# xiyichen/smplify-x-partial

Hardware: AMD Instinct MI355X
Metric: fitted frames/sec (higher is better)
Workload: dtype f32; 1 GPU; configs[1]: 256 synthetic frames/GPU, body-only K=25, camera + 5-stage L-BFGS (fit_smplx_smplifyx.yaml, use_vposer=False); frames_per_gpu=256, lbs_mode=dense, gemm_columns_per_gpu=256, parallelism=frames sharded, dp1, closure_evals_per_frame_max=4429, non_finite=0

## Files before the change

### smplify-x-partial_amd/csrc/closure_body.h

```cpp
#pragma once
#include "closure_math.h"
#include "closure_lds.h"
#pragma clang fp contract(on)

#define MARK(i) do { if (D.dbg && blockIdx.x == 0 && threadIdx.x == 0 && D.dbg[62] <= D.dbg[61]) { D.dbg[i] = clock64(); \
        if ((i) == 0) D.dbg[17] = wall_clock64(); if ((i) == 16) D.dbg[18] = wall_clock64(); } } while (0)

#define FOR_CT(w, N) _Pragma("unroll") for (int w##_i = 0; w##_i < ((N) + CT - 1) / CT; ++w##_i)             \
                         if (const int w = t + w##_i * CT; w < (N))

struct NoUpstream {};
struct ExtUpstream {
    const float* djoints;
    int has_dverts;
    float* gc;
};

struct OwnOperands {
    __device__ __forceinline__ int tid() const { return threadIdx.x; }
    __device__ __forceinline__ const float* featR(const BatchDev& D) const { return D.featR; }
    __device__ __forceinline__ float* featR_w(const BatchDev& D) const { return D.featR_w; }
    __device__ __forceinline__ float* AT_w(const BatchDev& D) const { return D.AT_w; }
};
struct OperandSets {
    const float* r; float* fw; float* aw; int t;
    __device__ __forceinline__ int tid() const { return t; }
    __device__ __forceinline__ const float* featR(const BatchDev&) const { return r; }
    __device__ __forceinline__ float* featR_w(const BatchDev&) const { return fw; }
    __device__ __forceinline__ float* AT_w(const BatchDev&) const { return aw; }
};

template <class LDS, class SW, class EXT = NoUpstream, class OPS = OwnOperands>
__device__ __forceinline__ void closure_body(LDS& S, const DevModel& M, const BatchDev& D,
                                             const VarList* __restrict__ vls, const SW* __restrict__ sws,
                                             const ClosureArgs& args, const int b, typename LDS::real_t* gflat,
                                             typename LDS::real_t* fout, const EXT& ext = EXT{}, const OPS ops = OPS{}) {
    using Real = typename LDS::real_t;
    constexpr bool F64 = std::is_same<Real, double>::value;
    constexpr bool kExt = !std::is_same<EXT, NoUpstream>::value;
    static_assert(!kExt || !F64, "the external-upstream sweep is fp32");
    constexpr int CT = LDS::kThreads;
    const int t = ops.tid();
    const int lane = t & 63, wv = t >> 6;
    const ParLayout& L = D.L;
    const BatchCfgDev& C = D.cfg;

    const bool self_uvp = !F64 && args.use_dense_verts == 2 && M.n_uniq > 0 && M.n_uniq <= LDS::kMaxItems;
    const int stage = __builtin_amdgcn_readfirstlane((args.stage_override != -2) ? args.stage_override : D.stage[b]);
    if constexpr (!kExt) { if (stage >= C.n_stages && !args.forward_only) return; }
    const bool cam_stage = (stage < 0);
    const SW sw = (kExt || cam_stage || args.forward_only) ? SW{} : sws[stage];

    const int cls = (kExt || cam_stage || args.forward_only) ? 2 : ((sw.face_jw != 0.f) ? 2 : ((sw.hand_jw != 0.f) ? 1 : 0));
    const int KL = __builtin_amdgcn_readfirstlane(cls == 2 ? M.K : C.kl[cls]);
    const int NIL = __builtin_amdgcn_readfirstlane(cls == 2 ? M.n_items : C.nil[cls]);

    MARK(0);
    constexpr bool HAS_VP = !std::is_same<decltype(S.V), EmptyLDS>::value;
    constexpr int RIF = (LDS::kMaxItems <= SFX_SMALL_ITEMS) ? SFX_RIF_SMALL : SFX_RIF_BIG;
    constexpr int FWD_PREFIX = (int)(offsetof(LDS, vp) / sizeof(float));
    static_assert(F64 || (FWD_PREFIX % 4 == 0 && FWD_PREFIX + 96 + 2 * VP_H + 128 + 64 <= SFX_FWD_N), "forward-state blob layout");
    static_assert(offsetof(LDS, Ad) % sizeof(fwd_t) == 0 && offsetof(LDS, cd) % sizeof(fwd_t) == 0, "forward-precision members");
    const bool reuse = !F64 && args.reuse_fwd != 0;
    float* fwd = D.fwd ? D.fwd + (size_t)b * SFX_FWD_N : nullptr;
    const Real* xsrc;
    if constexpr (F64) xsrc = (args.from_X ? D.X64 : D.Xt64) + (size_t)b * SFX_NPAR_MAX;
    else xsrc = (args.from_X ? D.X : D.Xt) + (size_t)b * SFX_NPAR_MAX;
    if (!reuse) {
        if (args.x_lds) { for (int i = t; i < L.npar; i += CT) S.x[i] = args.x_lds[i]; }
        else lds_fill_async<CT>(S.x, xsrc, L.npar * (int)(sizeof(Real) / 4));
    }
    if (!args.keep_tables) {
    static_assert(SFX_META_N % 4 == 0 && FD_N % 4 == 0 && offsetof(LDS, meta) % 16 == 0 && offsetof(LDS, fd) % 16 == 0, "16-byte copies");
    lds_fill_async16<CT>(S.meta, M.meta, SFX_META_N / 4);
    lds_fill_async16<CT>(S.fd, D.fd + (size_t)b * FD_N, FD_N / 4);
    const int ns = M.n_static_items;
    lds_fill_async<CT>(S.ivid, M.item_vid, ns); lds_fill_async<CT>(S.iw, M.item_w, ns); lds_fill_async<CT>(S.uslot, M.item_uslot, ns);
    lds_fill_async<CT>(S.vt, M.item_vt, ns * 3);
    lds_fill_async<CT>(S.wj, M.item_wj, ns * SFX_NW); lds_fill_async<CT>(S.ww, M.item_ww, ns * SFX_NW);
    if (M.n_sj <= LDS::kMaxItems * SFX_NW) {
        lds_fill_async<CT>(S.sjs, M.sj_start, SFX_J + 1);
        lds_fill_async<CT>(S.sji, M.sj_item, M.n_sj); lds_fill_async<CT>(S.sjw, M.sj_w, M.n_sj);
    }
    }
    if (reuse) {
        static_assert(F64 || offsetof(LDS, lut_row) == offsetof(LDS, lh45) + 2 * SFX_NHAND * sizeof(float), "hand poses + LUT row are one run");
        lds_fill_async16<CT>(&S, fwd, FWD_PREFIX / 4);
        const float* ex = fwd + FWD_PREFIX;
        lds_fill_async<CT>(S.lh45, ex, 2 * SFX_NHAND + 1);
        if constexpr (HAS_VP) if (C.use_vposer) {
            const float* vx = ex + 96;
            static_assert(offsetof(VposerLDS, h2) == VP_H * sizeof(float) && offsetof(VposerLDS, o) == 2 * VP_H * sizeof(float), "h1 | h2 | o are one run");
            lds_fill_async16<CT>(S.V.h1, vx, (2 * VP_H + 128) / 4);
            lds_fill_async16<CT>(S.V.body, vx + 2 * VP_H + 128, 64 / 4);
        }
    }
    for (int i = t; i < SFX_KD_PAD; i += CT) { if (!reuse) S.feat[i] = 0.f; S.dfeat[i] = 0.f; }
    for (int i = t; i < SFX_NPAR_MAX; i += CT) S.gc[i] = 0.f;
    for (int i = t; i < 168; i += CT) S.dpose[i] = 0.f;
    if constexpr (!F64) {
        if (self_uvp) self_blend_offsets(M.uniq_dirs, M.n_uniq, ops.featR(D) + (size_t)args.self_col * SFX_KD_PAD, S.dvert, wv, CT / 64, lane);
    }
    lds_dma_wait();
    __syncthreads();
    const Real* bodypose = S.x + L.emb;
    if constexpr (HAS_VP) {
        if (C.use_vposer && !reuse) {
            vposer_forward<CT>(S.V, M, S.x + L.emb, S.T);
            if (t < 63) D.bodypose[(size_t)b * 63 + t] = S.V.body[t];
        }
        if (C.use_vposer) bodypose = S.V.body;
    }
  if (!reuse) {

    MARK(1);
    if (t < SFX_POSE) {
        Real v;
        if (t < 3) v = S.x[L.go + t];
        else if (t < 66) v = bodypose[t - 3];
        else if (t < 69) v = S.x[L.jaw + t - 66];
        else if (t < 72) v = S.x[L.leye + t - 69];
        else if (t < 75) v = S.x[L.reye + t - 72];
        else {
            const bool left = t < 120;
            const int c = left ? t - 75 : t - 120;
            const float* comp = left ? M.comp_l : M.comp_r;
            const Real* pc = S.x + (left ? L.lh : L.rh);
            v = 0.f;
            for (int i = 0; i < L.NPCA; ++i) v += pc[i] * comp[i * SFX_NHAND + c];
            if (left) S.lh45[c] = v; else S.rh45[c] = v;
        }
        S.full_pose[t] = v + M.pose_mean[t];
    }
    if (t < M.S) S.feat[t] = (t < L.NB) ? S.x[L.betas + t] : S.x[L.expr + t - L.NB];
// ... 79 lines not shown
            float rel[9] = {1, 0, 0, 0, 1, 0, 0, 0, 1};
            const int chain[5] = {12, 9, 6, 3, 0};
            for (int q = 0; q < 5; ++q) {
                const Real* Rk = &S.R[chain[q] * 9];
                float o[9];
                for (int i = 0; i < 3; ++i)
                    for (int j = 0; j < 3; ++j)
                        o[i * 3 + j] = Rk[i * 3] * rel[j] + Rk[i * 3 + 1] * rel[3 + j] + Rk[i * 3 + 2] * rel[6 + j];
                for (int e = 0; e < 9; ++e) rel[e] = o[e];
            }
            const float sy = sqrtf(rel[0] * rel[0] + rel[3] * rel[3]);
            const float ang = atan2f(-rel[6], sy);
            float deg = (-ang) * 180.0f / 3.14159265358979323846f;
            deg = fminf(deg, 39.f);
            const int y = (int)rintf(deg);
            row = (y < -39) ? 78 : ((y < 0) ? (39 - y) : y);
        }
        S.lut_row = row;
    }
    __syncthreads();

  }
    MARK(4);
    if (!F64 && args.export_dense) {
        const int slot = D.slot[b];
        if (t < SFX_KD_PAD / 4) reinterpret_cast<float4*>(ops.featR_w(D) + (size_t)slot * SFX_KD_PAD)[t] = reinterpret_cast<const float4*>(S.feat)[t];
        MARK(17);
        for (int i = t; i < SFX_J * 12; i += CT) {
            const int j = i / 12, e = i % 12;
            ops.AT_w(D)[((size_t)e * SFX_JPAD + j) * D.Bpad + slot] = S.A[i];
        }
        MARK(18);
        if (args.forward_only == 2) {
            if (fwd) {
                const float* sp = reinterpret_cast<const float*>(&S);
                for (int i = t; i < FWD_PREFIX / 4; i += CT)
                    reinterpret_cast<float4*>(fwd)[i] = reinterpret_cast<const float4*>(sp)[i];
                float* ex = fwd + FWD_PREFIX;
                if (t < SFX_NHAND) { ex[t] = S.lh45[t]; ex[SFX_NHAND + t] = S.rh45[t]; }
                if (t == 64) ex[2 * SFX_NHAND] = __int_as_float(S.lut_row);
                if constexpr (HAS_VP) if (C.use_vposer) {
                    float* vx = ex + 96;
                    for (int i = t; i < VP_H; i += CT) { vx[i] = S.V.h1[i]; vx[VP_H + i] = S.V.h2[i]; }
                    if (t < 128) vx[2 * VP_H + t] = S.V.o[t];
                    if (t < 64) vx[2 * VP_H + 128 + t] = S.V.body[t];
                }
            }
            MARK(19);
            return;
        }
    }

    MARK(5);
    const int NI = NIL;
    const bool dyn_live = NI > M.n_static_items;
    const bool dyn_lds = dyn_live && M.dynp_js != nullptr && M.n_dyn_items <= LDS::kMaxDyn;
    if (dyn_live) {
        const int ns = M.n_static_items, nd = M.n_dyn_items;
        const size_t ro = (size_t)S.lut_row * nd;
        lds_fill_async<CT>(S.ivid + ns, M.dynp_vid + ro, nd); lds_fill_async<CT>(S.iw + ns, M.dynp_w + ro, nd);
        lds_fill_async<CT>(S.vt + ns * 3, M.dynp_vt + ro * 3, nd * 3);
        if (M.dynp_us) lds_fill_async<CT>(S.uslot + ns, M.dynp_us + ro, nd);
        lds_fill_async<CT>(S.wj + ns * SFX_NW, M.dynp_wj + ro * SFX_NW, nd * SFX_NW);
        lds_fill_async<CT>(S.ww + ns * SFX_NW, M.dynp_ww + ro * SFX_NW, nd * SFX_NW);
        if (dyn_lds) {
            lds_fill_async<CT>(S.djs, M.dynp_js + (size_t)S.lut_row * (SFX_J + 1), SFX_J + 1);
            lds_fill_async<CT>(S.dji, M.dynp_ji + ro * SFX_NW, nd * SFX_NW); lds_fill_async<CT>(S.djw, M.dynp_jw + ro * SFX_NW, nd * SFX_NW);
        }
        lds_dma_wait();
        __syncthreads();
    }
    auto items_forward = [&](const int ib, const int ni) {
    if constexpr (F64) {
        const double* fe = S.feat;
        double fa[4], fb[4];
#pragma unroll
        for (int c = 0; c < 4; ++c) { fa[c] = fe[4 * lane + c]; fb[c] = fe[256 + 4 * lane + c]; }
        const int nrow = ni * 3, rb = ib * 3;
        const int rot = (int)((blockIdx.x * 40u) % (unsigned)nrow);
        for (int w0 = wv * RIF; w0 < nrow; w0 += (CT / 64) * RIF) {
            float4 da[RIF], db[RIF];
            int myw, myrow;
            {
                const int u = lane < RIF ? lane : 0;
                int w = ((w0 + u < nrow) ? w0 + u : w0) + rot;
                w = w >= nrow ? w - nrow : w;
                w += rb;
                myw = w;
                myrow = S.ivid[w / 3] * 3 + w % 3;
            }
#pragma unroll
            for (int u = 0; u < RIF; ++u) {
                const int r = __builtin_amdgcn_readlane(myrow, u);
                const float4* row = reinterpret_cast<const float4*>(M.dirsT + (size_t)r * SFX_KD_PAD);
                da[u] = row[lane]; db[u] = row[64 + lane];
            }
#pragma unroll
            for (int u = 0; u < RIF; ++u) {
                const int w = __builtin_amdgcn_readlane(myw, u);
                double acc = fa[0] * (double)da[u].x + fa[1] * (double)da[u].y + fa[2] * (double)da[u].z + fa[3] * (double)da[u].w +
// ... 557 lines not shown
```

### smplify-x-partial_amd/csrc/closure_lds.h

```cpp
#pragma once
#include "closure_math.h"
#pragma clang fp contract(on)
#include "vposer.h"

__device__ __forceinline__ void red_put_int(float& r, int n) { r = __int_as_float(n); }
__device__ __forceinline__ void red_put_int(double& r, int n) { r = (double)n; }
__device__ __forceinline__ int red_get_int(float r) { return __float_as_int(r); }
__device__ __forceinline__ int red_get_int(double r) { return (int)r; }

#ifndef SFX_BIG_THREADS
#define SFX_BIG_THREADS 512
#endif
#define SFX_MAX_THREADS 512

struct EmptyLDS {};

typedef __attribute__((address_space(3))) void* sfx_lds_vp;
typedef const __attribute__((address_space(1))) void* sfx_glb_vp;
template <int CT>
__device__ __forceinline__ void lds_fill_async(void* lds_dst, const void* gsrc, const int n_dwords) {
    const int lane = threadIdx.x & 63, wv = threadIdx.x >> 6;
    const char* g = reinterpret_cast<const char*>(gsrc);
    char* l = reinterpret_cast<char*>(lds_dst);
    for (int base = wv * 64; base < n_dwords; base += CT) {
        const int i = base + lane;
        if (i < n_dwords) __builtin_amdgcn_global_load_lds((sfx_glb_vp)(g + 4 * (size_t)i), (sfx_lds_vp)(l + 4 * base), 4, 0, 0);
    }
}
__device__ __forceinline__ void lds_dma_wait() { __builtin_amdgcn_s_waitcnt(0x0F70); }
template <int CT>
__device__ __forceinline__ void lds_fill_async16(void* lds_dst, const void* gsrc, const int n16) {
    const int lane = threadIdx.x & 63, wv = threadIdx.x >> 6;
    const char* g = reinterpret_cast<const char*>(gsrc);
    char* l = reinterpret_cast<char*>(lds_dst);
    for (int base = wv * 64; base < n16; base += CT) {
        const int i = base + lane;
        if (i < n16) __builtin_amdgcn_global_load_lds((sfx_glb_vp)(g + 16 * (size_t)i), (sfx_lds_vp)(l + 16 * base), 16, 0, 0);
    }
}

typedef float sfx_f32x4 __attribute__((ext_vector_type(4)));
[[maybe_unused]] static __device__ __forceinline__ void self_blend_offsets(const float* __restrict__ uniq_dirs, const int n_uniq, const float* __restrict__ arow,
                                                                           float* out, const int wv, const int nw, const int lane) {
    constexpr int NCH = SFX_KD_PAD / SFX_DENSE_KC, KS = SFX_DENSE_KC / 4;
    constexpr int NG = 4, GS = NG * KS;
    static_assert(NCH % NG == 0 && KS % 4 == 0 && NCH * KS == 128, "operand groups; DevModel.uniq_dirs holds 128 steps per unit");
    const int jl = lane & 15, kq = lane >> 4;
    const int nunit = ((n_uniq + 15) / 16) * 3;
    for (int unit = wv; unit < nunit; unit += nw) {
        const int tile = unit / 3, co = unit - tile * 3;
        const int u = tile * 16 + jl;
        const float4* pb = reinterpret_cast<const float4*>(uniq_dirs) + (size_t)unit * (NCH * KS / 4) * 64 + lane;
        const float* pa = arow + kq;
        float a[NCH * KS];
        float4 bv[2][GS / 4];
#pragma unroll
        for (int c = 0; c < NCH; ++c)
#pragma unroll
            for (int ks = 0; ks < KS; ++ks) a[c * KS + ks] = pa[SFX_DENSE_KCHUNK(c) * SFX_DENSE_KC + ks * 4];
#define SELF_LOAD(g, buf) _Pragma("unroll") for (int q = 0; q < GS / 4; ++q) bv[buf][q] = pb[((g) * (GS / 4) + q) * 64];
        sfx_f32x4 acc = {0.f, 0.f, 0.f, 0.f};
        SELF_LOAD(0, 0)
#pragma unroll
        for (int g = 0; g < NCH / NG; ++g) {
            if (g + 1 < NCH / NG) { SELF_LOAD(g + 1, (g + 1) & 1) }
// ... 82 lines not shown
```

### smplify-x-partial_amd/csrc/fused.hip

```cpp
#include "closure_body.h"
#include "lbfgs_body.h"

#ifndef SFX_SETS_SMALL8
#define SFX_SETS_SMALL8 3
#endif
#ifndef SFX_TICK_OCC
#define SFX_TICK_OCC 2
#endif

template <class LDS>
__global__ __launch_bounds__(LDS::kThreads, LDS::kBlocksPerCU)
void k_fit_rows(DevModel M, BatchDev D, const VarList* __restrict__ vls, const StageW* __restrict__ sws,
                int first_stage, int last_stage, int max_ticks) {
    __shared__ LDS S;
    __shared__ float gflat[SFX_NVAR_MAX];
    __shared__ float fval;
    __shared__ float s_al[SFX_HIST_MAX + 2 * LB_BS];
    __shared__ OptScal st;
    const int b = blockIdx.x;
    ClosureArgs a{};
    a.stage_override = -2;
    for (int it = 0; it < max_ticks; ++it) {
        if (D.stage[b] > last_stage) break;
        closure_body(S, M, D, vls, sws, a, b, gflat, &fval);
// ... 82 lines not shown
    if (D.dbg && threadIdx.x == 0) {
        const long long dt = wall_clock64() - wc0;
        atomicMax((unsigned long long*)&D.dbg[58], (unsigned long long)dt);
        atomicAdd((unsigned long long*)&D.dbg[59], (unsigned long long)dt);
        atomicAdd((unsigned long long*)&D.dbg[60], 1ull);
    }
}

__global__ __launch_bounds__(FrameLDSSmall8::kThreads, 1)
void k_tick_dense_multi(DevModel M, BatchDev D, const VarList* __restrict__ vls, const StageW* __restrict__ sws,
                        int first_stage, int last_stage, TickSets sets, int R) {
    using LDS = FrameLDSSmall8;
    constexpr int CTK = LDS::kThreads;
    __shared__ LDS S;
    __shared__ float gflat[SFX_NVAR_MAX];
    __shared__ float fval;
    __shared__ float s_al[SFX_HIST_MAX + 2 * LB_BS];
    __shared__ OptScal st;
    __shared__ __align__(16) float s_pf[2048];
    __shared__ __align__(16) VarList s_vl[2];
    __shared__ int s_stage;
    __shared__ float* s_featR[SFX_TICK_ROUNDS + 1];
    __shared__ float* s_AT[SFX_TICK_ROUNDS + 1];
    const int b = D.act ? D.act[blockIdx.x] : blockIdx.x;
    const int slot = D.slot[b];
    const int self_col = __builtin_amdgcn_readfirstlane(M.n_uniq > 0 ? slot : 0);
    const bool stamp = D.dbg && blockIdx.x == 0 && threadIdx.x == 0;
    if (stamp) { D.dbg[62] += 1; if (D.dbg[62] <= D.dbg[61]) D.dbg[24] = clock64(); }
    if (threadIdx.x == 0) {
#pragma unroll
        for (int q = 0; q <= SFX_TICK_ROUNDS; ++q) { s_featR[q] = sets.featR[q]; s_AT[q] = sets.AT[q]; }
    }
    __syncthreads();
    int r = 0;
#pragma clang loop unroll(disable)
    for (bool live = D.stage[b] <= last_stage; live && r < R; ++r) {
        if (r) __syncthreads();
        int t = threadIdx.x;
        asm volatile("" : "+v"(t));
        const OperandSets ops{s_featR[r], s_featR[r + 1], s_AT[r + 1], t};
        ClosureArgs a{};
        a.stage_override = -2; a.use_dense_verts = 2; a.reuse_fwd = 1; a.keep_tables = r > 0; a.self_col = self_col;
        lds_fill_async16<CTK>(s_pf, D.vec + (size_t)b * NVEC * SFX_NVAR_MAX, NVEC * SFX_NVAR_MAX / 4);
        lds_fill_async16<CTK>(s_pf + NVEC * SFX_NVAR_MAX, D.X + (size_t)b * SFX_NPAR_MAX, SFX_NPAR_MAX / 4);
        lds_fill_async16<CTK>(s_pf + NVEC * SFX_NVAR_MAX + SFX_NPAR_MAX, D.Xt + (size_t)b * SFX_NPAR_MAX, SFX_NPAR_MAX / 4);
        lds_fill_async<CTK>(&st, &(reinterpret_cast<const OptState*>(D.opt) + b)->s, (int)(sizeof(OptScal) / 4));
        if (r == 0) lds_fill_async<CTK>(s_vl, vls, (int)(2 * sizeof(VarList) / 4));
        closure_body(S, M, D, vls, sws, a, b, gflat, &fval, NoUpstream{}, ops);
        __syncthreads();
        if (t < 64)
            lbfgs_tick_body<SFX_SETS_SMALL8, true>(M, D, s_vl, first_stage, last_stage, 0, 0, b, t, s_al, st, s_pf, &fval, gflat, &s_stage);
        __syncthreads();
        if (stamp && r == 0 && D.dbg[62] <= D.dbg[61]) { D.dbg[25] = clock64(); for (int i = 0; i < 17; ++i) D.dbg[40 + i] = D.dbg[i]; }
        const int stage_now = s_stage;
        if (stage_now > last_stage) { live = false; break; }
        ClosureArgs e{};
        e.stage_override = stage_now; e.export_dense = 1; e.forward_only = 2; e.keep_tables = 1;
        e.x_lds = s_pf + NVEC * SFX_NVAR_MAX + SFX_NPAR_MAX;
        closure_body(S, M, D, vls, sws, e, b, nullptr, nullptr, NoUpstream{}, ops);
        if (stamp && r == 0 && D.dbg[62] <= D.dbg[61]) D.dbg[26] = clock64();
    }
    if (r == R) return;
    const float4* const f0 = reinterpret_cast<const float4*>(s_featR[r] + (size_t)slot * SFX_KD_PAD);
    const float* const a0 = s_AT[r];
    for (int q = r + 1; q <= R; ++q) {
        if (threadIdx.x < SFX_KD_PAD / 4) reinterpret_cast<float4*>(s_featR[q] + (size_t)slot * SFX_KD_PAD)[threadIdx.x] = f0[threadIdx.x];
        for (int i = threadIdx.x; i < 12 * SFX_JPAD; i += CTK) s_AT[q][(size_t)i * D.Bpad + slot] = a0[(size_t)i * D.Bpad + slot];
    }
}

__global__ __launch_bounds__(256)
void k_uvp_self(DevModel M, BatchDev D, float* __restrict__ out) {
    const int col = blockIdx.x;
    self_blend_offsets(M.uniq_dirs, M.n_uniq, D.featR + (size_t)col * SFX_KD_PAD, out + (size_t)col * M.n_uniq * 3,
                       threadIdx.x >> 6, 4, threadIdx.x & 63);
}
void launch_uvp_self(const DevModel& M, const BatchDev& D, float* out, hipStream_t s) {
    if (D.cfg.B <= 0 || M.n_uniq <= 0) return;
    hipLaunchKernelGGL(k_uvp_self, dim3(D.cfg.B), dim3(256), 0, s, M, D, out);
}

void launch_fit_rows(const DevModel& M, const BatchDev& D, const VarList* vl_dev, const StageW* sw_dev,
                     int first_stage, int last_stage, int max_ticks, hipStream_t s) {
    if (sfx_small_closure(M, D))
        hipLaunchKernelGGL(k_fit_rows<FrameLDSSmall>, dim3(D.cfg.B), dim3(FrameLDSSmall::kThreads), 0, s, M, D, vl_dev, sw_dev, first_stage, last_stage, max_ticks);
    else
        hipLaunchKernelGGL(k_fit_rows<FrameLDS>, dim3(D.cfg.B), dim3(FrameLDS::kThreads), 0, s, M, D, vl_dev, sw_dev, first_stage, last_stage, max_ticks);
}
enum TickShape { TICK_SMALL8, TICK_SMALL_CU, TICK_SMALL_OCC };
static TickShape tick_small_shape(int grid) {
    static const int n_cu = [] { hipDeviceProp_t p; int dev = 0; (void)hipGetDevice(&dev); return hipGetDeviceProperties(&p, dev) == hipSuccess ? p.multiProcessorCount : 256; }();
#ifdef SFX_LAB
    static const bool t256 = [] { const char* e = getenv("SFX_TICK_THREADS"); return e && atoi(e) == 256; }();
#else
    constexpr bool t256 = false;
// ... 29 lines not shown
```

### smplify-x-partial_amd/csrc/host/inspect.hip

```cpp
#include "host.h"

#include <string>

#ifdef SFX_LAB
extern "C" int sfx_debug_phase_clocks(sfx_batch* b, int32_t stage, int64_t* out ) {
    if (!b) { sfx_set_error("null batch"); return -1; }
    if (refuse_f64(b, "sfx_debug_phase_clocks")) return -1;
    DevAlloc scratch;
    long long* d = scratch.zeros<long long>(64);
    if (scratch.failed) { (void)hipGetLastError(); sfx_set_error("out of device memory"); return -2; }
    { const long long freeze = 1 << 30; SFX_CHECK(hipMemcpy(d + 61, &freeze, sizeof(freeze), hipMemcpyHostToDevice)); }
    b->D.dbg = d;
    ClosureArgs a{}; a.stage_override = stage; a.from_X = 1;
    launch_closure(b->m->M, b->D, b->vl_dev, b->sw_dev, a, 0);
    launch_closure(b->m->M, b->D, b->vl_dev, b->sw_dev, a, 0);
    const hipError_t es = hipDeviceSynchronize();
    b->D.dbg = nullptr;
    SFX_CHECK(es);
    long long h[64];
    SFX_CHECK(hipMemcpy(h, d, sizeof(h), hipMemcpyDeviceToHost));
    for (int i = 0; i < 32; ++i) out[i] = h[i];
    return 0;
}
#endif

extern "C" int sfx_batch_debug_read(sfx_batch* b, const char* name, float* out, int64_t n_out) {
    if (!b || !name || !out) { sfx_set_error("null argument"); return -1; }
    const BatchDev& D = b->D; const int B = D.cfg.B, V = b->m->M.V;
    const std::string k(name);
    SFX_CHECK(hipDeviceSynchronize());
    auto plain = [&](const float* src, size_t per) -> int {
        if (!src) { sfx_set_error("buffer '%s' is not allocated in this batch", name); return -1; }
        if ((int64_t)(per * B) != n_out) { sfx_set_error("'%s' holds %zu floats, caller asked for %lld", name, per * B, (long long)n_out); return -1; }
        SFX_CHECK(hipMemcpy(out, src, per * B * sizeof(float), hipMemcpyDeviceToHost));
        return 0;
    };
    if (k == "verts") return plain(D.verts, (size_t)V * 3);
    if (k == "vposed") return plain(D.vposed, (size_t)V * 3);
    if (k == "pen_dverts") return plain(D.pen_dverts, (size_t)V * 3);
    if (k == "pen_dfeat") return plain(D.pen_dfeat, SFX_KD_PAD);
    if (k == "pen_dA") return plain(D.pen_dA, (size_t)SFX_J * 12);
    if (k == "pen_loss") return plain(D.pen_loss, 1);
    if (k == "uvp") return plain(D.uvp, (size_t)b->m->M.n_uniq * 3);
    if (k == "uvp_self") {
        const size_t n = (size_t)B * b->m->M.n_uniq * 3;
        if ((int64_t)n != n_out) { sfx_set_error("'%s' holds %zu floats, caller asked for %lld", name, n, (long long)n_out); return -1; }
        if (!n) return 0;
        if (!D.featR) { sfx_set_error("buffer '%s' is not allocated in this batch", name); return -1; }
        DevAlloc scratch;
        float* d = scratch.zeros<float>(n);
        if (!d) { (void)hipGetLastError(); sfx_set_error("out of device memory"); return -2; }
        launch_uvp_self(b->m->M, D, d, nullptr);
        SFX_CHECK(hipDeviceSynchronize());
        SFX_CHECK(hipMemcpy(out, d, n * sizeof(float), hipMemcpyDeviceToHost));
        return 0;
    }
    if (k == "A" || k == "feat") {
        const size_t rows = k == "A" ? (size_t)12 * SFX_JPAD : SFX_KD_PAD, per = k == "A" ? (size_t)12 * SFX_J : SFX_KD_PAD;
        if ((int64_t)(per * B) != n_out) { sfx_set_error("'%s' holds %zu floats, caller asked for %lld", name, per * B, (long long)n_out); return -1; }
        std::vector<float> h(rows * D.Bpad);
        SFX_CHECK(hipMemcpy(h.data(), k == "A" ? D.AT : D.featR, h.size() * sizeof(float), hipMemcpyDeviceToHost));
        for (int i = 0; i < B; ++i) {
            if (k == "A") { for (int e = 0; e < 12; ++e) for (int j = 0; j < SFX_J; ++j) out[((size_t)i * 12 + e) * SFX_J + j] = h[((size_t)e * SFX_JPAD + j) * D.Bpad + i]; }
            else for (int q = 0; q < SFX_KD_PAD; ++q) out[(size_t)i * SFX_KD_PAD + q] = h[(size_t)i * SFX_KD_PAD + q];
        }
        return 0;
    }
    sfx_set_error("unknown buffer '%s'", name);
    return -1;
}

extern "C" int sfx_lbfgs_two_loop(const float* S, const float* Y, int32_t count, int32_t history_size, const float* g, float* d_out) {
    if (!S || !Y || !g || !d_out || count < 1 || history_size > SFX_HIST_MAX) { sfx_set_error("sfx_lbfgs_two_loop: bad arguments"); return -1; }
    const int rc = debug_two_loop(S, Y, count, history_size > 0 ? history_size : SFX_HIST, g, d_out);
    if (rc) { sfx_set_error("sfx_lbfgs_two_loop: HIP error"); return -1; }
    return 0;
// ... 127 lines not shown
```

### smplify-x-partial_amd/csrc/lbfgs_body.h

```cpp
#pragma once
#include "sfx_internal.h"
#include "wave_ops.h"
#pragma clang fp contract(off)
#define LB_BS 8
#define LB_SYNC() do { __builtin_amdgcn_fence(__ATOMIC_SEQ_CST, "workgroup"); __builtin_amdgcn_wave_barrier(); } while (0)

enum { PH_ENTRY = 0, PH_BRACKET = 1, PH_ZOOM = 2 };
enum { A_NONE = 0, A_ENTRY, A_ITER_HEAD, A_ZOOM_NEXT, A_FINISH_LS, A_END_STEP, A_FINISH_STAGE };

struct Sc { double v; int t; };
__device__ __forceinline__ Sc P(double v) { Sc s; s.v = v; s.t = 0; return s; }
__device__ __forceinline__ Sc T(float v) { Sc s; s.v = (double)v; s.t = 1; return s; }
__device__ __forceinline__ Sc sc_add(Sc a, Sc b) { return (a.t | b.t) ? T((float)a.v + (float)b.v) : P(a.v + b.v); }
__device__ __forceinline__ Sc sc_sub(Sc a, Sc b) { return (a.t | b.t) ? T((float)a.v - (float)b.v) : P(a.v - b.v); }
__device__ __forceinline__ Sc sc_mul(Sc a, Sc b) { return (a.t | b.t) ? T((float)a.v * (float)b.v) : P(a.v * b.v); }
__device__ __forceinline__ Sc sc_div(Sc a, Sc b) { return (a.t | b.t) ? T((float)a.v / (float)b.v) : P(a.v / b.v); }
__device__ __forceinline__ bool sc_lt(Sc a, Sc b) { return (a.t | b.t) ? ((float)a.v < (float)b.v) : (a.v < b.v); }
__device__ __forceinline__ bool sc_le(Sc a, Sc b) { return (a.t | b.t) ? ((float)a.v <= (float)b.v) : (a.v <= b.v); }
__device__ __forceinline__ bool sc_gt(Sc a, Sc b) { return (a.t | b.t) ? ((float)a.v > (float)b.v) : (a.v > b.v); }
__device__ __forceinline__ bool sc_ge(Sc a, Sc b) { return (a.t | b.t) ? ((float)a.v >= (float)b.v) : (a.v >= b.v); }
__device__ __forceinline__ Sc sc_pmax(Sc a, Sc b) { return sc_gt(b, a) ? b : a; }
__device__ __forceinline__ Sc sc_pmin(Sc a, Sc b) { return sc_lt(b, a) ? b : a; }
__device__ __forceinline__ Sc sc_abs(Sc a) { a.v = fabs(a.v); return a; }
__device__ __forceinline__ Sc sc_neg(Sc a) { a.v = -a.v; return a; }
// ... 307 lines not shown
            if (m < 7) acc = fmaf(cc[m], X.bnd[m], acc);
        }
#pragma unroll
        for (int c = 0; c < 8; ++c) lb_axpy(r, cc[c], X.all[c]);
    };
#define LB_LD2(X, b_) lb_load<1>(X, (b_), n, head, hY, hS, gst->syb, gst->ro, s_alp, true, lane, R)
    {
        int i0 = 0, k = 0;
        const int last = max(n - 1, 0);
        if constexpr (SETS == 3) {
        LB_LD2(A, i0); LB_LD2(B, min(i0 + 8, last));
        for (; k + 3 <= nb; k += 3) {
            LB_LD2(C, min(i0 + 16, last)); LB_PIN(); up(A); LB_PIN(); i0 += 8;
            LB_LD2(A, min(i0 + 16, last)); LB_PIN(); up(B); LB_PIN(); i0 += 8;
            LB_LD2(B, min(i0 + 16, last)); LB_PIN(); up(C); LB_PIN(); i0 += 8;
        }
        if (k < nb) { up(A); LB_PIN(); if (k + 1 < nb) { up(B); LB_PIN(); } }
        } else {
        LB_LD2(A, i0);
        for (; k + 2 <= nb; k += 2) {
            LB_LD2(B, min(i0 + 8, last)); LB_PIN(); up(A); LB_PIN(); i0 += 8;
            LB_LD2(A, min(i0 + 8, last)); LB_PIN(); up(B); LB_PIN(); i0 += 8;
        }
        if (k < nb) { up(A); LB_PIN(); }
        }
    }
#undef LB_LD2
#undef LB_PIN
#undef LB_RL
    Lane3 out; out.v[0] = r.a.x; out.v[1] = r.a.y; out.v[2] = r.b;
    return out;
}

template <int SETS, bool PF = false>
__device__ __forceinline__ void lbfgs_tick_wave0(const DevModel& M, const BatchDev& D, const VarList* __restrict__ vls,
                                                 int first_stage, int last_stage, int init, int step_mode,
                                                 const int b, const int lane, float* s_al, OptScal& s_state, float* s_work,
                                                 const float* f_src, const float* g_src, int* stage_out = nullptr) {
    const BatchCfgDev& C = D.cfg;
    OptState* gst = reinterpret_cast<OptState*>(D.opt) + b;
    int stage = D.stage[b];
    float* Xg = D.X + (size_t)b * SFX_NPAR_MAX;
    float* Xtg = D.Xt + (size_t)b * SFX_NPAR_MAX;
    float* vecg = D.vec + (size_t)b * NVEC * SFX_NVAR_MAX;
#ifdef SFX_RING_CONST
    const int R = SFX_HIST, hrows = R + 8;
#else
    const int R = C.hist_ring, hrows = R + 8;
#endif
    float* hY = D.hist + (size_t)b * 2 * hrows * SFX_NVAR_MAX;
    float* hS = hY + (size_t)hrows * SFX_NVAR_MAX;
#define VEC(k) (vec + (k) * SFX_NVAR_MAX)

    if (init == 1) {
        const OptScal s = fresh_state();
        stage = first_stage;
        if (lane == 0) {
            D.stage[b] = stage;
            gst->s = s;
            D.orient_pass[b] = 0;
            int both = 0;
            if (C.side_thsh > 0.f) {
                const float* g2 = D.gt + (size_t)b * M.K * 2;
                const float dx = g2[2 * C.lsh] - g2[2 * C.rsh], dy = g2[2 * C.lsh + 1] - g2[2 * C.rsh + 1];
                both = sqrtf(dx * dx + dy * dy) < C.side_thsh;
            }
            D.try_both[b] = both;
        }
        for (int i = lane; i < hrows * LB_BROW; i += 64) { gst->syb[i] = 0.f; gst->syt[i] = 0.f; }
        for (int q = lane; q < 1 + SFX_MAX_STAGES; q += 64) {
            if (q >= first_stage + 1 && q <= last_stage + 1) {
                D.stage_evals[(size_t)b * (1 + SFX_MAX_STAGES) + q] = 0;
                D.stage_ref_evals[(size_t)b * (1 + SFX_MAX_STAGES) + q] = 0;
            }
// ... 327 lines not shown
                    }
                    LB_SYNC();
                    if (lane == 0) {
                        float fl[3];
                        flipped_orientation(D.gocam + (size_t)b * 4, fl);
                        X[L.go] = fl[0]; X[L.go + 1] = fl[1]; X[L.go + 2] = fl[2];
                        D.orient_pass[b] = 1;
                    }
                    if (L.has_bodyp && lane < 63) X[L.bodyp + lane] = X[L.emb + lane];
                    LB_SYNC();
                    stage = 0;
                } else {
                    const float l0 = D.stage_loss[so + C.n_stages], l1 = res;
                    if (l0 < l1) {
                        for (int i = lane; i < SFX_NPAR_MAX; i += 64) X[i] = X0[i];
                    } else if (lane == 0) {
                        for (int q = 1; q <= C.n_stages; ++q) D.stage_loss[so + q] = D.stage_loss2[so + q];
                    }
                    if (lane == 0) D.orient_pass[b] = 2;
                    LB_SYNC();
                }
            }
            if (lane == 0) D.stage[b] = stage;
            s = fresh_state();
            for (int i = lane; i < SFX_NPAR_MAX; i += 64) Xt[i] = X[i];
            act = A_NONE;
            break;
        }
        default: act = A_NONE; break;
        }
    }
    TMARK(6);
    LB_SYNC();
#pragma unroll
    for (int k = 0; k < NVEC; ++k) st3_full(vecg + k * SFX_NVAR_MAX, ld3_raw(vec, (unsigned)k * SFX_NVAR_MAX, lane), lane);
    reinterpret_cast<float4*>(Xg)[lane] = reinterpret_cast<const float4*>(X)[lane];
    reinterpret_cast<float4*>(Xtg)[lane] = reinterpret_cast<const float4*>(Xt)[lane];
    if (lane == 0) gst->s = s_state;
    if (PF && lane == 0) *stage_out = stage;
    TMARK(7);
#undef TMARK
#undef TRACE
#undef VEC
}

template <int SETS, bool PF = false>
__device__ __forceinline__ void lbfgs_tick_body(const DevModel& M, const BatchDev& D, const VarList* __restrict__ vls,
                                                int first_stage, int last_stage, int init, int step_mode,
                                                const int b, const int tid, float* s_al, OptScal& s_state, float* s_work,
                                                const float* f_src, const float* g_src, int* stage_out = nullptr) {
    if (tid >= 64) return;
    lbfgs_tick_wave0<SETS, PF>(M, D, vls, first_stage, last_stage, init, step_mode, b, tid, s_al, s_state, s_work, f_src, g_src, stage_out);
}


#pragma clang fp contract(fast)
```

Baseline: 673.4 frames/s.

## Keep L-BFGS and forward state resident in LDS across fused tick rounds

In the fused multi-round tick kernel, optimizer vectors, X/Xt, the opt state and the var list are now loaded into LDS once before the round loop instead of every round. Later rounds reuse the forward state already in LDS instead of reloading it from global memory, and the global forward-state blob is stored only on the final round or on early exit. The stage is passed down rather than re-read from global memory, and the tick's global write-back is moved into a block-wide helper that uses all threads. This cuts global memory traffic per round, but correctness now depends on LDS contents surviving between rounds and on the write-back being done on every exit path.

After: 684.4 frames/s (median of 6 runs). +1.6%, better.

```diff
diff --git a/smplify-x-partial_amd/csrc/closure_body.h b/smplify-x-partial_amd/csrc/closure_body.h
--- a/smplify-x-partial_amd/csrc/closure_body.h
+++ b/smplify-x-partial_amd/csrc/closure_body.h
@@ -21,14 +21,37 @@
     __device__ __forceinline__ const float* featR(const BatchDev& D) const { return D.featR; }
     __device__ __forceinline__ float* featR_w(const BatchDev& D) const { return D.featR_w; }
     __device__ __forceinline__ float* AT_w(const BatchDev& D) const { return D.AT_w; }
+    __device__ __forceinline__ constexpr bool fwd_resident() const { return false; }
+    __device__ __forceinline__ constexpr bool fwd_store() const { return true; }
 };
 struct OperandSets {
     const float* r; float* fw; float* aw; int t;
+    bool resident, store;
     __device__ __forceinline__ int tid() const { return t; }
     __device__ __forceinline__ const float* featR(const BatchDev&) const { return r; }
     __device__ __forceinline__ float* featR_w(const BatchDev&) const { return fw; }
     __device__ __forceinline__ float* AT_w(const BatchDev&) const { return aw; }
+    __device__ __forceinline__ bool fwd_resident() const { return resident; }
+    __device__ __forceinline__ bool fwd_store() const { return store; }
 };
+
+template <class LDS>
+__device__ __forceinline__ void save_forward_state(const LDS& S, float* fwd, const int t, const bool use_vposer) {
+    constexpr int CT = LDS::kThreads;
+    constexpr int FWD_PREFIX = (int)(offsetof(LDS, vp) / sizeof(float));
+    const float* sp = reinterpret_cast<const float*>(&S);
+    for (int i = t; i < FWD_PREFIX / 4; i += CT)
+        reinterpret_cast<float4*>(fwd)[i] = reinterpret_cast<const float4*>(sp)[i];
+    float* ex = fwd + FWD_PREFIX;
+    if (t < SFX_NHAND) { ex[t] = S.lh45[t]; ex[SFX_NHAND + t] = S.rh45[t]; }
+    if (t == 64) ex[2 * SFX_NHAND] = __int_as_float(S.lut_row);
+    if constexpr (!std::is_same<decltype(S.V), EmptyLDS>::value) if (use_vposer) {
+        float* vx = ex + 96;
+        for (int i = t; i < VP_H; i += CT) { vx[i] = S.V.h1[i]; vx[VP_H + i] = S.V.h2[i]; }
+        if (t < 128) vx[2 * VP_H + t] = S.V.o[t];
+        if (t < 64) vx[2 * VP_H + 128 + t] = S.V.body[t];
+    }
+}
 
 template <class LDS, class SW, class EXT = NoUpstream, class OPS = OwnOperands>
 __device__ __forceinline__ void closure_body(LDS& S, const DevModel& M, const BatchDev& D,
@@ -68,38 +91,41 @@
     else xsrc = (args.from_X ? D.X : D.Xt) + (size_t)b * SFX_NPAR_MAX;
     if (!reuse) {
         if (args.x_lds) { for (int i = t; i < L.npar; i += CT) S.x[i] = args.x_lds[i]; }
-        else lds_fill_async<CT>(S.x, xsrc, L.npar * (int)(sizeof(Real) / 4));
+        else lds_fill_async<CT>(S.x, xsrc, L.npar * (int)(sizeof(Real) / 4), t);
     }
     if (!args.keep_tables) {
     static_assert(SFX_META_N % 4 == 0 && FD_N % 4 == 0 && offsetof(LDS, meta) % 16 == 0 && offsetof(LDS, fd) % 16 == 0, "16-byte copies");
-    lds_fill_async16<CT>(S.meta, M.meta, SFX_META_N / 4);
-    lds_fill_async16<CT>(S.fd, D.fd + (size_t)b * FD_N, FD_N / 4);
+    lds_fill_async16<CT>(S.meta, M.meta, SFX_META_N / 4, t);
+    lds_fill_async16<CT>(S.fd, D.fd + (size_t)b * FD_N, FD_N / 4, t);
     const int ns = M.n_static_items;
-    lds_fill_async<CT>(S.ivid, M.item_vid, ns); lds_fill_async<CT>(S.iw, M.item_w, ns); lds_fill_async<CT>(S.uslot, M.item_uslot, ns);
-    lds_fill_async<CT>(S.vt, M.item_vt, ns * 3);
-    lds_fill_async<CT>(S.wj, M.item_wj, ns * SFX_NW); lds_fill_async<CT>(S.ww, M.item_ww, ns * SFX_NW);
+    lds_fill_async<CT>(S.ivid, M.item_vid, ns, t); lds_fill_async<CT>(S.iw, M.item_w, ns, t); lds_fill_async<CT>(S.uslot, M.item_uslot, ns, t);
+    lds_fill_async<CT>(S.vt, M.item_vt, ns * 3, t);
+    lds_fill_async<CT>(S.wj, M.item_wj, ns * SFX_NW, t); lds_fill_async<CT>(S.ww, M.item_ww, ns * SFX_NW, t);
     if (M.n_sj <= LDS::kMaxItems * SFX_NW) {
-        lds_fill_async<CT>(S.sjs, M.sj_start, SFX_J + 1);
-        lds_fill_async<CT>(S.sji, M.sj_item, M.n_sj); lds_fill_async<CT>(S.sjw, M.sj_w, M.n_sj);
-    }
-    }
-    if (reuse) {
+        lds_fill_async<CT>(S.sjs, M.sj_start, SFX_J + 1, t);
+        lds_fill_async<CT>(S.sji, M.sj_item, M.n_sj, t); lds_fill_async<CT>(S.sjw, M.sj_w, M.n_sj, t);
+    }
+    }
+    if (reuse && !ops.fwd_resident()) {
         static_assert(F64 || offsetof(LDS, lut_row) == offsetof(LDS, lh45) + 2 * SFX_NHAND * sizeof(float), "hand poses + LUT row are one run");
-        lds_fill_async16<CT>(&S, fwd, FWD_PREFIX / 4);
+        lds_fill_async16<CT>(&S, fwd, FWD_PREFIX / 4, t);
         const float* ex = fwd + FWD_PREFIX;
-        lds_fill_async<CT>(S.lh45, ex, 2 * SFX_NHAND + 1);
+        lds_fill_async<CT>(S.lh45, ex, 2 * SFX_NHAND + 1, t);
         if constexpr (HAS_VP) if (C.use_vposer) {
             const float* vx = ex + 96;
             static_assert(offsetof(VposerLDS, h2) == VP_H * sizeof(float) && offsetof(VposerLDS, o) == 2 * VP_H * sizeof(float), "h1 | h2 | o are one run");
-            lds_fill_async16<CT>(S.V.h1, vx, (2 * VP_H + 128) / 4);
-            lds_fill_async16<CT>(S.V.body, vx + 2 * VP_H + 128, 64 / 4);
+            lds_fill_async16<CT>(S.V.h1, vx, (2 * VP_H + 128) / 4, t);
+            lds_fill_async16<CT>(S.V.body, vx + 2 * VP_H + 128, 64 / 4, t);
         }
     }
     for (int i = t; i < SFX_KD_PAD; i += CT) { if (!reuse) S.feat[i] = 0.f; S.dfeat[i] = 0.f; }
     for (int i = t; i < SFX_NPAR_MAX; i += CT) S.gc[i] = 0.f;
     for (int i = t; i < 168; i += CT) S.dpose[i] = 0.f;
     if constexpr (!F64) {
-        if (self_uvp) self_blend_offsets(M.uniq_dirs, M.n_uniq, ops.featR(D) + (size_t)args.self_col * SFX_KD_PAD, S.dvert, wv, CT / 64, lane);
+        if (self_uvp) {
+            if (reuse && ops.fwd_resident()) self_blend_offsets(M.uniq_dirs, M.n_uniq, reinterpret_cast<const float*>(S.feat), S.dvert, wv, CT / 64, lane);
+            else self_blend_offsets(M.uniq_dirs, M.n_uniq, ops.featR(D) + (size_t)args.self_col * SFX_KD_PAD, S.dvert, wv, CT / 64, lane);
+        }
     }
     lds_dma_wait();
     __syncthreads();
@@ -245,20 +271,7 @@
         }
         MARK(18);
         if (args.forward_only == 2) {
-            if (fwd) {
-                const float* sp = reinterpret_cast<const float*>(&S);
-                for (int i = t; i < FWD_PREFIX / 4; i += CT)
-                    reinterpret_cast<float4*>(fwd)[i] = reinterpret_cast<const float4*>(sp)[i];
-                float* ex = fwd + FWD_PREFIX;
-                if (t < SFX_NHAND) { ex[t] = S.lh45[t]; ex[SFX_NHAND + t] = S.rh45[t]; }
-                if (t == 64) ex[2 * SFX_NHAND] = __int_as_float(S.lut_row);
-                if constexpr (HAS_VP) if (C.use_vposer) {
-                    float* vx = ex + 96;
-                    for (int i = t; i < VP_H; i += CT) { vx[i] = S.V.h1[i]; vx[VP_H + i] = S.V.h2[i]; }
-                    if (t < 128) vx[2 * VP_H + t] = S.V.o[t];
-                    if (t < 64) vx[2 * VP_H + 128 + t] = S.V.body[t];
-                }
-            }
+            if (fwd && ops.fwd_store()) save_forward_state(S, fwd, t, C.use_vposer != 0);
             MARK(19);
             return;
         }
@@ -271,14 +284,14 @@
     if (dyn_live) {
         const int ns = M.n_static_items, nd = M.n_dyn_items;
         const size_t ro = (size_t)S.lut_row * nd;
-        lds_fill_async<CT>(S.ivid + ns, M.dynp_vid + ro, nd); lds_fill_async<CT>(S.iw + ns, M.dynp_w + ro, nd);
-        lds_fill_async<CT>(S.vt + ns * 3, M.dynp_vt + ro * 3, nd * 3);
-        if (M.dynp_us) lds_fill_async<CT>(S.uslot + ns, M.dynp_us + ro, nd);
-        lds_fill_async<CT>(S.wj + ns * SFX_NW, M.dynp_wj + ro * SFX_NW, nd * SFX_NW);
-        lds_fill_async<CT>(S.ww + ns * SFX_NW, M.dynp_ww + ro * SFX_NW, nd * SFX_NW);
+        lds_fill_async<CT>(S.ivid + ns, M.dynp_vid + ro, nd, t); lds_fill_async<CT>(S.iw + ns, M.dynp_w + ro, nd, t);
+        lds_fill_async<CT>(S.vt + ns * 3, M.dynp_vt + ro * 3, nd * 3, t);
+        if (M.dynp_us) lds_fill_async<CT>(S.uslot + ns, M.dynp_us + ro, nd, t);
+        lds_fill_async<CT>(S.wj + ns * SFX_NW, M.dynp_wj + ro * SFX_NW, nd * SFX_NW, t);
+        lds_fill_async<CT>(S.ww + ns * SFX_NW, M.dynp_ww + ro * SFX_NW, nd * SFX_NW, t);
         if (dyn_lds) {
-            lds_fill_async<CT>(S.djs, M.dynp_js + (size_t)S.lut_row * (SFX_J + 1), SFX_J + 1);
-            lds_fill_async<CT>(S.dji, M.dynp_ji + ro * SFX_NW, nd * SFX_NW); lds_fill_async<CT>(S.djw, M.dynp_jw + ro * SFX_NW, nd * SFX_NW);
+            lds_fill_async<CT>(S.djs, M.dynp_js + (size_t)S.lut_row * (SFX_J + 1), SFX_J + 1, t);
+            lds_fill_async<CT>(S.dji, M.dynp_ji + ro * SFX_NW, nd * SFX_NW, t); lds_fill_async<CT>(S.djw, M.dynp_jw + ro * SFX_NW, nd * SFX_NW, t);
         }
         lds_dma_wait();
         __syncthreads();
diff --git a/smplify-x-partial_amd/csrc/closure_lds.h b/smplify-x-partial_amd/csrc/closure_lds.h
--- a/smplify-x-partial_amd/csrc/closure_lds.h
+++ b/smplify-x-partial_amd/csrc/closure_lds.h
@@ -18,8 +18,8 @@
 typedef __attribute__((address_space(3))) void* sfx_lds_vp;
 typedef const __attribute__((address_space(1))) void* sfx_glb_vp;
 template <int CT>
-__device__ __forceinline__ void lds_fill_async(void* lds_dst, const void* gsrc, const int n_dwords) {
-    const int lane = threadIdx.x & 63, wv = threadIdx.x >> 6;
+__device__ __forceinline__ void lds_fill_async(void* lds_dst, const void* gsrc, const int n_dwords, const int tid = threadIdx.x) {
+    const int lane = tid & 63, wv = tid >> 6;
     const char* g = reinterpret_cast<const char*>(gsrc);
     char* l = reinterpret_cast<char*>(lds_dst);
     for (int base = wv * 64; base < n_dwords; base += CT) {
@@ -29,8 +29,8 @@
 }
 __device__ __forceinline__ void lds_dma_wait() { __builtin_amdgcn_s_waitcnt(0x0F70); }
 template <int CT>
-__device__ __forceinline__ void lds_fill_async16(void* lds_dst, const void* gsrc, const int n16) {
-    const int lane = threadIdx.x & 63, wv = threadIdx.x >> 6;
+__device__ __forceinline__ void lds_fill_async16(void* lds_dst, const void* gsrc, const int n16, const int tid = threadIdx.x) {
+    const int lane = tid & 63, wv = tid >> 6;
     const char* g = reinterpret_cast<const char*>(gsrc);
     char* l = reinterpret_cast<char*>(lds_dst);
     for (int base = wv * 64; base < n16; base += CT) {
diff --git a/smplify-x-partial_amd/csrc/fused.hip b/smplify-x-partial_amd/csrc/fused.hip
--- a/smplify-x-partial_amd/csrc/fused.hip
+++ b/smplify-x-partial_amd/csrc/fused.hip
@@ -138,35 +138,42 @@
         for (int q = 0; q <= SFX_TICK_ROUNDS; ++q) { s_featR[q] = sets.featR[q]; s_AT[q] = sets.AT[q]; }
     }
     __syncthreads();
-    int r = 0;
-#pragma clang loop unroll(disable)
-    for (bool live = D.stage[b] <= last_stage; live && r < R; ++r) {
-        if (r) __syncthreads();
-        int t = threadIdx.x;
-        asm volatile("" : "+v"(t));
-        const OperandSets ops{s_featR[r], s_featR[r + 1], s_AT[r + 1], t};
-        ClosureArgs a{};
-        a.stage_override = -2; a.use_dense_verts = 2; a.reuse_fwd = 1; a.keep_tables = r > 0; a.self_col = self_col;
+    int stage_now = D.stage[b];
+    if (stage_now <= last_stage) {
         lds_fill_async16<CTK>(s_pf, D.vec + (size_t)b * NVEC * SFX_NVAR_MAX, NVEC * SFX_NVAR_MAX / 4);
         lds_fill_async16<CTK>(s_pf + NVEC * SFX_NVAR_MAX, D.X + (size_t)b * SFX_NPAR_MAX, SFX_NPAR_MAX / 4);
         lds_fill_async16<CTK>(s_pf + NVEC * SFX_NVAR_MAX + SFX_NPAR_MAX, D.Xt + (size_t)b * SFX_NPAR_MAX, SFX_NPAR_MAX / 4);
         lds_fill_async<CTK>(&st, &(reinterpret_cast<const OptState*>(D.opt) + b)->s, (int)(sizeof(OptScal) / 4));
-        if (r == 0) lds_fill_async<CTK>(s_vl, vls, (int)(2 * sizeof(VarList) / 4));
+        lds_fill_async<CTK>(s_vl, vls, (int)(2 * sizeof(VarList) / 4));
+    }
+    int r = 0;
+    const bool live_at_entry = stage_now <= last_stage;
+#pragma clang loop unroll(disable)
+    for (bool live = live_at_entry; live && r < R; ++r) {
+        if (r) __syncthreads();
+        int t = threadIdx.x;
+        asm volatile("" : "+v"(t));
+        const OperandSets ops{s_featR[r], s_featR[r + 1], s_AT[r + 1], t, r > 0, r + 1 == R};
+        ClosureArgs a{};
+        a.stage_override = stage_now; a.use_dense_verts = 2; a.reuse_fwd = 1; a.keep_tables = r > 0; a.self_col = self_col;
         closure_body(S, M, D, vls, sws, a, b, gflat, &fval, NoUpstream{}, ops);
         __syncthreads();
         if (t < 64)
-            lbfgs_tick_body<SFX_SETS_SMALL8, true>(M, D, s_vl, first_stage, last_stage, 0, 0, b, t, s_al, st, s_pf, &fval, gflat, &s_stage);
+            lbfgs_tick_body<SFX_SETS_SMALL8, true, false>(M, D, s_vl, first_stage, last_stage, 0, 0, b, t, s_al, st, s_pf, &fval, gflat, &s_stage, stage_now);
         __syncthreads();
         if (stamp && r == 0 && D.dbg[62] <= D.dbg[61]) { D.dbg[25] = clock64(); for (int i = 0; i < 17; ++i) D.dbg[40 + i] = D.dbg[i]; }
-        const int stage_now = s_stage;
+        stage_now = __builtin_amdgcn_readfirstlane(s_stage);
         if (stage_now > last_stage) { live = false; break; }
         ClosureArgs e{};
         e.stage_override = stage_now; e.export_dense = 1; e.forward_only = 2; e.keep_tables = 1;
         e.x_lds = s_pf + NVEC * SFX_NVAR_MAX + SFX_NPAR_MAX;
         closure_body(S, M, D, vls, sws, e, b, nullptr, nullptr, NoUpstream{}, ops);
+        tick_write_back<CTK>(D, b, s_pf, st, t);
         if (stamp && r == 0 && D.dbg[62] <= D.dbg[61]) D.dbg[26] = clock64();
     }
     if (r == R) return;
+    if (live_at_entry) tick_write_back<CTK>(D, b, s_pf, st, (int)threadIdx.x);
+    if (r > 0 && D.fwd) save_forward_state(S, D.fwd + (size_t)b * SFX_FWD_N, (int)threadIdx.x, false);
     const float4* const f0 = reinterpret_cast<const float4*>(s_featR[r] + (size_t)slot * SFX_KD_PAD);
     const float* const a0 = s_AT[r];
     for (int q = r + 1; q <= R; ++q) {
diff --git a/smplify-x-partial_amd/csrc/host/inspect.hip b/smplify-x-partial_amd/csrc/host/inspect.hip
--- a/smplify-x-partial_amd/csrc/host/inspect.hip
+++ b/smplify-x-partial_amd/csrc/host/inspect.hip
@@ -42,6 +42,7 @@
     if (k == "pen_dA") return plain(D.pen_dA, (size_t)SFX_J * 12);
     if (k == "pen_loss") return plain(D.pen_loss, 1);
     if (k == "uvp") return plain(D.uvp, (size_t)b->m->M.n_uniq * 3);
+    if (k == "fwd") return plain(D.fwd, SFX_FWD_N);
     if (k == "uvp_self") {
         const size_t n = (size_t)B * b->m->M.n_uniq * 3;
         if ((int64_t)n != n_out) { sfx_set_error("'%s' holds %zu floats, caller asked for %lld", name, n, (long long)n_out); return -1; }
diff --git a/smplify-x-partial_amd/csrc/lbfgs_body.h b/smplify-x-partial_amd/csrc/lbfgs_body.h
--- a/smplify-x-partial_amd/csrc/lbfgs_body.h
+++ b/smplify-x-partial_amd/csrc/lbfgs_body.h
@@ -363,14 +363,15 @@
     return out;
 }
 
-template <int SETS, bool PF = false>
+template <int SETS, bool PF = false, bool WB = true>
 __device__ __forceinline__ void lbfgs_tick_wave0(const DevModel& M, const BatchDev& D, const VarList* __restrict__ vls,
                                                  int first_stage, int last_stage, int init, int step_mode,
                                                  const int b, const int lane, float* s_al, OptScal& s_state, float* s_work,
-                                                 const float* f_src, const float* g_src, int* stage_out = nullptr) {
+                                                 const float* f_src, const float* g_src, int* stage_out = nullptr,
+                                                 const int stage_in = -2) {
     const BatchCfgDev& C = D.cfg;
     OptState* gst = reinterpret_cast<OptState*>(D.opt) + b;
-    int stage = D.stage[b];
+    int stage = (PF && stage_in != -2) ? stage_in : D.stage[b];
     float* Xg = D.X + (size_t)b * SFX_NPAR_MAX;
     float* Xtg = D.Xt + (size_t)b * SFX_NPAR_MAX;
     float* vecg = D.vec + (size_t)b * NVEC * SFX_NVAR_MAX;
@@ -764,11 +765,13 @@
     }
     TMARK(6);
     LB_SYNC();
+    if constexpr (WB) {
 #pragma unroll
     for (int k = 0; k < NVEC; ++k) st3_full(vecg + k * SFX_NVAR_MAX, ld3_raw(vec, (unsigned)k * SFX_NVAR_MAX, lane), lane);
     reinterpret_cast<float4*>(Xg)[lane] = reinterpret_cast<const float4*>(X)[lane];
     reinterpret_cast<float4*>(Xtg)[lane] = reinterpret_cast<const float4*>(Xt)[lane];
     if (lane == 0) gst->s = s_state;
+    }
     if (PF && lane == 0) *stage_out = stage;
     TMARK(7);
 #undef TMARK
@@ -776,13 +779,29 @@
 #undef VEC
 }
 
-template <int SETS, bool PF = false>
+template <int CT>
+__device__ __forceinline__ void tick_write_back(const BatchDev& D, const int b, const float* s_work, const OptScal& s_state, const int t) {
+    constexpr int NV4 = NVEC * SFX_NVAR_MAX / 4, NX4 = SFX_NPAR_MAX / 4;
+    for (int i = t; i < NV4 + 2 * NX4; i += CT) {
+        const float4 v = reinterpret_cast<const float4*>(s_work)[i];
+        float4* dst = i < NV4 ? reinterpret_cast<float4*>(D.vec + (size_t)b * NVEC * SFX_NVAR_MAX) + i
+                    : i < NV4 + NX4 ? reinterpret_cast<float4*>(D.X + (size_t)b * SFX_NPAR_MAX) + (i - NV4)
+                                    : reinterpret_cast<float4*>(D.Xt + (size_t)b * SFX_NPAR_MAX) + (i - NV4 - NX4);
+        *dst = v;
+    }
+    int* gs = reinterpret_cast<int*>(&(reinterpret_cast<OptState*>(D.opt) + b)->s);
+    const int* ls = reinterpret_cast<const int*>(&s_state);
+    for (int i = t; i < (int)(sizeof(OptScal) / 4); i += CT) gs[i] = ls[i];
+}
+
+template <int SETS, bool PF = false, bool WB = true>
 __device__ __forceinline__ void lbfgs_tick_body(const DevModel& M, const BatchDev& D, const VarList* __restrict__ vls,
                                                 int first_stage, int last_stage, int init, int step_mode,
                                                 const int b, const int tid, float* s_al, OptScal& s_state, float* s_work,
-                                                const float* f_src, const float* g_src, int* stage_out = nullptr) {
+                                                const float* f_src, const float* g_src, int* stage_out = nullptr,
+                                                const int stage_in = -2) {
     if (tid >= 64) return;
-    lbfgs_tick_wave0<SETS, PF>(M, D, vls, first_stage, last_stage, init, step_mode, b, tid, s_al, s_state, s_work, f_src, g_src, stage_out);
+    lbfgs_tick_wave0<SETS, PF, WB>(M, D, vls, first_stage, last_stage, init, step_mode, b, tid, s_al, s_state, s_work, f_src, g_src, stage_out, stage_in);
 }
 
 
```
